# JialeTao/MRFA

Hardware: AMD Instinct MI355X
Metric: frames/sec (256x256 source+driving pair) fwd+bwd (higher is better)
Workload: dtype f32; 1 GPU; vox1.yaml MTIA (TokenPose_B) prior + DenseMotion + RaftFlow refinement, 256x256, bs=8/GPU, fwd+bwd+clip+Adam, train-mode BN, surrogate L1 loss; global_batch=8, parallelism=dp1, prior=mtia, background_predictor=False, sync_bn=False, launch=hipGraph, optimizer=FlatAdam (K20), mfma=bf16x6

## Files before the change

### mrfa_amd/csrc/common.h

```cpp
#pragma once
#include <hip/hip_runtime.h>
#include <stdio.h>
#include <string.h>
#include "mrfa_hip.h"

typedef float f32x16 __attribute__((ext_vector_type(16)));
typedef float f32x4 __attribute__((ext_vector_type(4)));

void mrfa_set_error(const char* fmt, ...);

struct MrfaTuning {
    int conv_small_env;
    int conv_small;
    int conv_halo, conv_halo_min_tiles, conv_halo_pr, conv_halo_phase, conv_halo_bn256, conv_halo_bn192, conv_halo_bn64_fill;
    int conv_lean, conv_lean_min_wgs, conv_lean_geo, gemm_lean;
    int wgrad_halo, wgrad_halo_min_wgs, wgrad_halo_target_wgs, wgrad_halo_phase, wgrad_lean;
    int conv_fewout3, attention_mfma, split_target_256;
};
extern MrfaTuning g_tune;

struct HaloGeo { int PR, BN; bool phase; };

enum class ConvFamily { lean, gemm_lean, small, halo, halo_dgrad, rows_split, rows_f32, refused };
struct ConvPlan {
    ConvFamily family;
    char error[256];
    long long M;
    int KT;
    int lean_geo, gemm_cfg, small_tm, small_tn;
    HaloGeo halo;
    int BM, BN, splitk;
    bool w8;
// ... 175 lines not shown
```

### mrfa_amd/csrc/conv_plan.hip

```cpp
#include "common.h"
#include <stdarg.h>
#include <stdlib.h>

namespace {
int env_int(const char* name, int dflt) { const char* e = getenv(name); return e ? atoi(e) : dflt; }
int env_on(const char* name) { const char* e = getenv(name); return !(e && e[0] == '0'); }
}

MrfaTuning g_tune = {
     env_on("MRFA_CONV_SMALL"),  1,
     env_on("MRFA_CONV_HALO"),  128,  0,  1,  1,
     1,  1,
     env_on("MRFA_CONV_LEAN"),  128,  -1,
     env_int("MRFA_GEMM_LEAN", 1),
     env_on("MRFA_WGRAD_HALO"),  192,  256,  1,
     env_on("MRFA_WGRAD_LEAN"),
     1,  env_on("MRFA_ATTENTION_MFMA"),  env_int("MRFA_SPLIT_TARGET_256", 1),
};

enum TuneKind { T_ON, T_INT, T_NONNEG, T_NONNEG_ON, T_LEVEL, T_POS };
static const struct { const char* key; int* field; TuneKind kind; } TUNING_KEYS[] = {
    {"conv_small", &g_tune.conv_small, T_ON},
    {"conv_halo", &g_tune.conv_halo, T_ON},
    {"conv_halo_min_tiles", &g_tune.conv_halo_min_tiles, T_INT},
    {"conv_halo_pr", &g_tune.conv_halo_pr, T_INT},
    {"conv_halo_phase", &g_tune.conv_halo_phase, T_ON},
    {"conv_halo_bn256", &g_tune.conv_halo_bn256, T_ON},
    {"conv_halo_bn192", &g_tune.conv_halo_bn192, T_ON},
    {"conv_halo_bn64_fill", &g_tune.conv_halo_bn64_fill, T_ON},
    {"conv_lean", &g_tune.conv_lean, T_ON},
    {"conv_lean_min_wgs", &g_tune.conv_lean_min_wgs, T_NONNEG},
    {"conv_lean_geo", &g_tune.conv_lean_geo, T_INT},
    {"gemm_lean", &g_tune.gemm_lean, T_LEVEL},
    {"wgrad_halo", &g_tune.wgrad_halo, T_ON},
    {"wgrad_halo_min_wgs", &g_tune.wgrad_halo_min_wgs, T_NONNEG},
    {"wgrad_halo_target_wgs", &g_tune.wgrad_halo_target_wgs, T_POS},
    {"wgrad_halo_phase", &g_tune.wgrad_halo_phase, T_NONNEG_ON},
    {"wgrad_lean", &g_tune.wgrad_lean, T_ON},
    {"conv_fewout3", &g_tune.conv_fewout3, T_ON},
    {"attention_mfma", &g_tune.attention_mfma, T_ON},
};

extern "C" int mrfa_set_tuning(const char* key, int value) {
    if (!key) return -1;
    for (const auto& k : TUNING_KEYS) {
        if (strcmp(key, k.key)) continue;
        const int prev = *k.field;
        switch (k.kind) {
            case T_ON: *k.field = value != 0; break;
            case T_INT: *k.field = value; break;
            case T_NONNEG: if (value >= 0) *k.field = value; break;
            case T_NONNEG_ON: if (value >= 0) *k.field = value != 0; break;
            case T_LEVEL: if (value >= 0) *k.field = value > 2 ? 2 : value; break;
            case T_POS: if (value > 0) *k.field = value; break;
        }
// ... 202 lines not shown
```

### mrfa_amd/csrc/elementwise.hip

```cpp
#include "common.h"

namespace {

#define GRID_STRIDE(i, total) \
    for (long long i = blockIdx.x * (long long)blockDim.x + threadIdx.x; i < (total); i += (long long)gridDim.x * blockDim.x)

__global__ void avgpool2_fwd_kernel(const float* __restrict__ x, int ldx, int H, int W, int C, float* __restrict__ y, int ldy,
                                    long long total) {
    const int Ho = H / 2, Wo = W / 2;
    GRID_STRIDE(i, total) {
        const long long opix = i / C;
        const int c = (int)(i - opix * C);
        const int ox = (int)(opix % Wo);
        const long long t = opix / Wo;
        const int oy = (int)(t % Ho);
        const long long n = t / Ho;
        const size_t b = (((size_t)n * H + 2 * oy) * W + 2 * ox) * ldx + c;
        y[(size_t)opix * ldy + c] = 0.25f * (x[b] + x[b + ldx] + x[b + (size_t)W * ldx] + x[b + (size_t)(W + 1) * ldx]);
    }
}

__global__ void sumpool2_acc_kernel(const float* __restrict__ x, int ldx, int Ho, int Wo, int C, float* __restrict__ y, int ldy, float mul,
                                    long long total) {
    const int H = 2 * Ho, W = 2 * Wo;
// ... 99 lines not shown
            const float o = occ[(size_t)r * ldo];
            const float g = dy[(size_t)r * lddy + c];
            const float av = a[(size_t)r * lda + c];
            const float bv = b ? b[(size_t)r * ldb + c] : 0.f;
            if (da) da[(size_t)r * ldda + c] += g * o;
            if (db) db[(size_t)r * lddb + c] += g * (1.f - o);
            part = g * (av - bv);
        }
        if (docc) {
            part = wave_sum(part);
            if (lane == 0) atomicAdd(docc + (size_t)r * lddo, part);
        }
    }
}

__global__ __launch_bounds__(256) void colsum_kernel(const float* __restrict__ x, int ldx, long long rows, int C, float* __restrict__ out,
                                                    int rows_per_block) {
    __shared__ float red[4][64];
    const int lane = threadIdx.x & 63, wave = threadIdx.x >> 6;
    const int c = blockIdx.x * 64 + lane;
    const long long r0 = (long long)blockIdx.y * rows_per_block, r1 = min(rows, r0 + rows_per_block);
    float s = 0.f;
    if (c < C)
        for (long long r = r0 + wave; r < r1; r += 4) s += x[(size_t)r * ldx + c];
    red[wave][lane] = s;
    __syncthreads();
    if (wave == 0 && c < C) atomicAdd(out + c, red[0][lane] + red[1][lane] + red[2][lane] + red[3][lane]);
}

__global__ void antialias_kernel(const float* __restrict__ x, int C, int H, int W, const float* __restrict__ kern, int k, int stride,
// ... 77 lines not shown
}

extern "C" int mrfa_blend_fwd(void* stream, const float* a, int lda, const float* b, int ldb, const float* occ, int ldo, long long rows,
                              int C, float* y, int ldy) {
    MRFA_CHECK_ARG(a && occ && y && rows > 0 && C > 0, "blend_fwd: bad args");
    const long long total = rows * C;
    hipLaunchKernelGGL(blend_fwd_kernel, dim3(stream_grid(total, 256)), dim3(256), 0, (hipStream_t)stream, a, lda, b, ldb, occ, ldo, C, y,
                       ldy, total);
    MRFA_CHECK_LAUNCH("blend_fwd");
    return 0;
}

extern "C" int mrfa_blend_bwd(void* stream, const float* a, int lda, const float* b, int ldb, const float* occ, int ldo, const float* dy,
                              int lddy, long long rows, int C, float* da, int ldda, float* db, int lddb, float* docc, int lddo) {
    MRFA_CHECK_ARG(a && occ && dy && rows > 0 && C > 0, "blend_bwd: bad args");
    const long long waves = rows * cdiv(C, 64);
    hipLaunchKernelGGL(blend_bwd_kernel, dim3(stream_grid(waves * 64, 256)), dim3(256), 0, (hipStream_t)stream, a, lda, b, ldb, occ, ldo, dy,
                       lddy, rows, C, da, ldda, db, lddb, docc, lddo);
    MRFA_CHECK_LAUNCH("blend_bwd");
    return 0;
}

extern "C" int mrfa_colsum(void* stream, const float* x, int ldx, long long rows, int C, float* out) {
    MRFA_CHECK_ARG(x && out && rows > 0 && C > 0, "colsum: bad args");
    const int chunks = cdiv(C, 64);
    long long want = (1024 + chunks - 1) / chunks;
    long long rpb = (rows + want - 1) / want;
    if (rpb < 64) rpb = 64;
    dim3 grid(chunks, cdiv(rows, rpb));
    hipLaunchKernelGGL(colsum_kernel, grid, dim3(256), 0, (hipStream_t)stream, x, ldx, rows, C, out, (int)rpb);
// ... 15 lines not shown
```

### mrfa_amd/csrc/norm.hip

```cpp
#include "common.h"

namespace {

constexpr int CH = 64;
constexpr int NW = 4;

__global__ __launch_bounds__(256) void bn_stats_kernel(const float* __restrict__ x, int ldx, long long rows, int C,
                                                      double* __restrict__ stats, int rows_per_block) {
    __shared__ float red[2][NW][CH];
    const int lane = threadIdx.x & 63, wave = threadIdx.x >> 6;
    const int c = blockIdx.x * CH + lane;
    const long long r0 = (long long)blockIdx.y * rows_per_block;
    const long long r1 = min(rows, r0 + rows_per_block);
    float s1 = 0.f, s2 = 0.f;
    if (c < C) {
        for (long long r = r0 + wave; r < r1; r += NW) {
            const float v = x[(size_t)r * ldx + c];
            s1 += v;
            s2 += v * v;
        }
    }
    red[0][wave][lane] = s1;
    red[1][wave][lane] = s2;
    __syncthreads();
    if (wave == 0 && c < C) {
        double a = 0.0, b = 0.0;
        for (int w = 0; w < NW; ++w) { a += red[0][w][lane]; b += red[1][w][lane]; }
        double* st = stats + (size_t)((blockIdx.y + blockIdx.x) % MRFA_STATS_SLOTS) * 2 * C;
        atomicAdd(st + c, a);
        atomicAdd(st + C + c, b);
    }
}

__global__ void bn_finalize_kernel(const double* __restrict__ stats, long long count, const float* __restrict__ gamma,
                                   const float* __restrict__ beta, float* __restrict__ rmean, float* __restrict__ rvar,
                                   float momentum, float eps, int C, int train, int groups, float* __restrict__ scale,
                                   float* __restrict__ shift, float* __restrict__ mean_out, float* __restrict__ invstd_out) {
    chain_prio();
    const int c = blockIdx.x * blockDim.x + threadIdx.x;
    if (c >= C) return;
    float rm = rmean ? rmean[c] : 0.f, rv = rvar ? rvar[c] : 0.f;
    for (int g = 0; g < groups; ++g) {
        float mean, invstd;
        if (train) {
            const double* sg = stats + (size_t)g * MRFA_STATS_SLOTS * 2 * C;
// ... 64 lines not shown
    for (long long i = blockIdx.x * (long long)blockDim.x + threadIdx.x; i < total4; i += (long long)gridDim.x * blockDim.x) {
        const long long opix = i / c4;
        const int c = (int)(i - opix * c4) * 4;
        const int gc = gpix ? (int)(opix / gpix) * p.C + c : c;
        const f32x4 sc = *reinterpret_cast<const f32x4*>(p.scale + gc), sh = *reinterpret_cast<const f32x4*>(p.shift + gc);
        f32x4 v = *reinterpret_cast<const f32x4*>(p.x + (size_t)opix * p.ldx + c) * sc + sh;
        if (RES) v += *reinterpret_cast<const f32x4*>(p.res + (size_t)opix * p.ldr + c);
        if (p.relu) {
#pragma unroll
            for (int k = 0; k < 4; ++k) v[k] = fmaxf(v[k], 0.f);
        }
        *reinterpret_cast<f32x4*>(p.y + (size_t)opix * p.ldy + c) = v;
    }
}

__device__ __forceinline__ int red_slots(unsigned row_blocks) {
    return row_blocks >= 64 ? MRFA_STATS_SLOTS : (row_blocks >= 16 ? 8 : 1);
}

struct GroupSpan {
    int g;
    unsigned by, row_blocks;
    long long cnt, r0, r1;
};
__device__ __forceinline__ GroupSpan group_span(const mrfa_bnbwd_params& p, long long rows, int rows_per_block) {
    GroupSpan s;
    const int G = p.groups > 1 ? p.groups : 1;
    s.row_blocks = gridDim.y / G;
    s.g = blockIdx.y / s.row_blocks;
    s.by = blockIdx.y - s.g * s.row_blocks;
// ... 78 lines not shown
    if (PHASE == 1) {
        red[0][wave][lane] = s1;
        red[1][wave][lane] = s2;
        __syncthreads();
        if (wave == 0 && c_ok) {
            double a = 0.0, b = 0.0;
            for (int w = 0; w < NW; ++w) { a += red[0][w][lane]; b += red[1][w][lane]; }
            double* rd = red_g + (size_t)((gs.by + blockIdx.x) % red_slots(gs.row_blocks)) * 2 * p.C;
            atomicAdd(rd + c, a);
            atomicAdd(rd + p.C + c, b);
        }
    }
}


template <int PHASE, int MODE>
__device__ __forceinline__ void bn_bwd_body(const mrfa_bnbwd_params& p, long long rows, int rows_per_block, float (&red)[2][16][CH],
                                            double (&redsum)[2][CH]) {
    constexpr bool POOL = MODE == 2, BLEND = MODE == 3, RES = MODE == 1;
    const int lane = threadIdx.x & 63, wave = threadIdx.x >> 6;
    const int cg = lane & 15, rsub = lane >> 4;
    const int slot = wave * 4 + rsub;
    const int c = blockIdx.x * CH + cg * 4;
    const bool c_ok = c < p.C;
    const GroupSpan gs = group_span(p, rows, rows_per_block);
    const int gc = gs.g * p.C + c;
    double* const red_g = p.red + (size_t)gs.g * MRFA_STATS_SLOTS * 2 * p.C;
    if (PHASE == 2 && (p.train || p.dbeta || p.dgamma)) {
        const int nslots = p.red_all ? MRFA_STATS_SLOTS : red_slots(gs.row_blocks);
        const int q = threadIdx.x & 3, col = (threadIdx.x >> 2) & 63;
        const int cc = blockIdx.x * CH + col;
// ... 72 lines not shown
                    if (st) {
#pragma unroll
                        for (int k = 0; k < 4; ++k) {
                            s1[k] += du[k];
                            s2[k] += du[k] * (xv[u][k] - mean[k]) * invstd[k];
                        }
                    }
                } else if (st) {
#pragma unroll
                    for (int k = 0; k < 4; ++k)
                        cur[u][k] += p.train ? gi[k] * (du[k] - k1[k] - (xv[u][k] - mean[k]) * invstd[k] * k2[k]) : du[k] * sc[k];
                    *reinterpret_cast<f32x4*>(p.dx + (size_t)rr[u] * p.lddx + c) = cur[u];
                }
            }
        }
    } else
    for (long long r = r0 + slot; r < r1; r += 16) {
        long long opix = r;
        float gmul = 1.f;
        if (POOL) {
            const int xx = (int)(r % p.W);
            const long long t = r / p.W;
            const int yy = (int)(t % p.H);
            const long long n = t / p.H;
            opix = ((long long)n * Ho + (yy >> 1)) * Wo + (xx >> 1);
            gmul = 0.25f;
        }
        f32x4 du = {0, 0, 0, 0}, xv = du;
        float docc_part = 0.f;
        if (c_ok) {
// ... 66 lines not shown
            red[0][slot][cg * 4 + k] = s1[k];
            red[1][slot][cg * 4 + k] = s2[k];
        }
        __syncthreads();
        const int cc = blockIdx.x * CH + threadIdx.x;
        if (threadIdx.x < CH && cc < p.C) {
            double a = 0.0, b = 0.0;
            for (int w = 0; w < 16; ++w) { a += red[0][w][threadIdx.x]; b += red[1][w][threadIdx.x]; }
            double* rd = red_g + (size_t)((gs.by + blockIdx.x) % red_slots(gs.row_blocks)) * 2 * p.C;
            atomicAdd(rd + cc, a);
            atomicAdd(rd + p.C + cc, b);
        }
    }
}

template <int PHASE, int MODE>
__global__ __launch_bounds__(256) void bn_act_bwd_vec_kernel(const mrfa_bnbwd_params p, long long rows, int rows_per_block) {
    chain_prio();
    __shared__ float red[2][16][CH];
    __shared__ double redsum[2][CH];
    bn_bwd_body<PHASE, MODE>(p, rows, rows_per_block, red, redsum);
}

__global__ void bn_param_grad_kernel(const double* __restrict__ red, float* __restrict__ dgamma, float* __restrict__ dbeta, int C, int nslots) {
    chain_prio();
    const int c = blockIdx.x * blockDim.x + threadIdx.x;
    if (c >= C) return;
    double t1 = 0.0, t2 = 0.0;
    for (int s = 0; s < nslots; ++s) { t1 += red[(size_t)s * 2 * C + c]; t2 += red[(size_t)s * 2 * C + C + c]; }
    if (dbeta) atomicAdd(dbeta + c, (float)t1);
    if (dgamma) atomicAdd(dgamma + c, (float)t2);
}

extern "C" int mrfa_bn_param_grad_groups(void* stream, const double* red, int C, int groups, float* dgamma, float* dbeta) {
    MRFA_CHECK_ARG(red && C > 0 && groups >= 1 && (dgamma || dbeta), "bn_param_grad: bad args");
    hipLaunchKernelGGL(bn_param_grad_kernel, dim3(cdiv(C, 256)), dim3(256), 0, (hipStream_t)stream, red, dgamma, dbeta, C, groups * MRFA_STATS_SLOTS);
// ... 11 lines not shown
    if (target > 1024) target = 1024;
    long long want = (target + chunks - 1) / chunks;
    long long rpb = (rows + want - 1) / want;
    if (rpb < 64) rpb = 64;
    if (rpb > 4096) rpb = 4096;
    return (int)rpb;
}

}

extern "C" int mrfa_bn_stats(void* stream, const float* x, int ldx, long long rows, int C, double* stats) {
    MRFA_CHECK_ARG(x && stats && rows > 0 && C > 0, "bn_stats: bad args");
    const int chunks = cdiv(C, CH);
    const int rpb = pick_rows_per_block(rows, chunks, C);
    dim3 grid(chunks, cdiv(rows, rpb));
    hipLaunchKernelGGL(bn_stats_kernel, grid, dim3(256), 0, (hipStream_t)stream, x, ldx, rows, C, stats, rpb);
    MRFA_CHECK_LAUNCH("bn_stats");
    return 0;
}

extern "C" int mrfa_bn_finalize(void* stream, const double* stats, long long count, const float* gamma, const float* beta,
                                float* running_mean, float* running_var, float momentum, float eps, int C, int train,
                                float* scale, float* shift, float* mean_out, float* invstd_out) {
    MRFA_CHECK_ARG(gamma && beta && scale && shift && C > 0, "bn_finalize: bad args");
    MRFA_CHECK_ARG(train ? stats != nullptr : (running_mean && running_var), "bn_finalize: missing statistics");
    hipLaunchKernelGGL(bn_finalize_kernel, dim3(cdiv(C, 256)), dim3(256), 0, (hipStream_t)stream, stats, count, gamma, beta,
                       running_mean, running_var, momentum, eps, C, train, 1, scale, shift, mean_out, invstd_out);
    MRFA_CHECK_LAUNCH("bn_finalize");
    return 0;
}
// ... 14 lines not shown
    MRFA_CHECK_ARG(p.x && p.y && p.scale && p.shift, "bn_act_fwd: null pointer");
    MRFA_CHECK_ARG(!p.pool || ((p.H % 2) == 0 && (p.W % 2) == 0), "bn_act_fwd: pool needs even H,W");
    MRFA_CHECK_ARG(!(p.pool && p.blend_a), "bn_act_fwd: pool and blend are exclusive");
    MRFA_CHECK_ARG(!(p.res && (p.pool || p.blend_a)), "bn_act_fwd: residual excludes pool and blend");
    MRFA_CHECK_ARG(p.groups <= 1 || (p.N % p.groups) == 0, "bn_act_fwd: %d statistic groups do not divide N = %d", p.groups, p.N);
    const long long opix = (long long)p.N * (p.pool ? p.H / 2 : p.H) * (p.pool ? p.W / 2 : p.W);
    const long long total = opix * p.C;
    if (!p.pool && !p.blend_a && (p.C % 4) == 0 && (p.ldx % 4) == 0 && (p.ldy % 4) == 0 && aligned16(p.x) && aligned16(p.y) && aligned16(p.scale) &&
        aligned16(p.shift) && (!p.res || ((p.ldr % 4) == 0 && aligned16(p.res)))) {
        const long long total4 = total / 4;
        if (p.res) hipLaunchKernelGGL((bn_act_fwd_vec_kernel<true>), dim3(stream_grid(total4, 256)), dim3(256), 0, (hipStream_t)stream, p, total4, p.C / 4);
        else hipLaunchKernelGGL((bn_act_fwd_vec_kernel<false>), dim3(stream_grid(total4, 256)), dim3(256), 0, (hipStream_t)stream, p, total4, p.C / 4);
        MRFA_CHECK_LAUNCH("bn_act_fwd(vec)");
        return 0;
    }
    hipLaunchKernelGGL(bn_act_fwd_kernel, dim3(stream_grid(total, 256)), dim3(256), 0, (hipStream_t)stream, p, total);
    MRFA_CHECK_LAUNCH("bn_act_fwd");
    return 0;
}

extern "C" int mrfa_bn_act_bwd(void* stream, const mrfa_bnbwd_params* pp) {
    const mrfa_bnbwd_params& p = *pp;
    MRFA_CHECK_ARG(p.x && p.dy && p.scale && p.shift && p.red, "bn_act_bwd: null pointer");
    MRFA_CHECK_ARG(!p.train || (p.mean && p.invstd && p.gamma), "bn_act_bwd: train mode needs mean/invstd/gamma");
    MRFA_CHECK_ARG(!(p.res && (p.pool || p.blend_a)) && !(p.dres && !p.res), "bn_act_bwd: residual excludes pool and blend");
    MRFA_CHECK_ARG(!(p.pool && p.blend_a), "bn_act_bwd: pool and blend are exclusive (one compile-time MODE per launch)");
    const int G = p.groups > 1 ? p.groups : 1;
    MRFA_CHECK_ARG((p.N % G) == 0, "bn_act_bwd: %d statistic groups do not divide N = %d", G, p.N);
    const long long rows = (long long)p.N * p.H * p.W;
    const int chunks = cdiv(p.C, CH);
    const int rpb = pick_rows_per_block(rows, chunks, p.C);
    dim3 grid(chunks, G * cdiv(rows / G, rpb));
    MRFA_CHECK_ARG(p.phase == 1 || p.phase == 2, "bn_act_bwd: phase %d", p.phase);
    const bool vec = (p.C % 4 == 0) && (p.ldx % 4 == 0) && (p.lddy % 4 == 0) && aligned16(p.x) && aligned16(p.dy) && aligned16(p.scale) &&
                     aligned16(p.shift) && (!p.mean || (aligned16(p.mean) && aligned16(p.invstd))) && (!p.gamma || aligned16(p.gamma)) &&
                     (p.phase == 1 || ((p.lddx % 4 == 0) && aligned16(p.dx))) &&
                     (!p.res || ((p.ldr % 4 == 0) && aligned16(p.res) && (!p.dres || ((p.lddr % 4 == 0) && aligned16(p.dres))))) &&
                     (!p.blend_a || ((p.lda % 4 == 0) && aligned16(p.blend_a) && (!p.dblend_a || ((p.ldda % 4 == 0) && aligned16(p.dblend_a)))));
    if (vec) {
        MRFA_CHECK_ARG(p.phase == 1 || p.dx != nullptr, "bn_act_bwd: phase 2 needs dx");
        const int mode = p.pool ? 2 : (p.blend_a ? 3 : (p.res ? 1 : 0));
#define BNB(PH, MD) hipLaunchKernelGGL((bn_act_bwd_vec_kernel<PH, MD>), grid, dim3(256), 0, (hipStream_t)stream, p, rows, rpb)
        if (p.phase == 1) { if (mode == 0) BNB(1, 0); else if (mode == 1) BNB(1, 1); else if (mode == 2) BNB(1, 2); else BNB(1, 3); }
        else { if (mode == 0) BNB(2, 0); else if (mode == 1) BNB(2, 1); else if (mode == 2) BNB(2, 2); else BNB(2, 3); }
#undef BNB
        MRFA_CHECK_LAUNCH("bn_act_bwd(vec)");
        return 0;
    }
    if (p.phase == 1) {
        hipLaunchKernelGGL((bn_act_bwd_kernel<1>), grid, dim3(256), 0, (hipStream_t)stream, p, rows, rpb);
    } else {
        MRFA_CHECK_ARG(p.dx != nullptr, "bn_act_bwd: phase 2 needs dx");
        hipLaunchKernelGGL((bn_act_bwd_kernel<2>), grid, dim3(256), 0, (hipStream_t)stream, p, rows, rpb);
        if (p.dgamma || p.dbeta) {
            hipLaunchKernelGGL(bn_param_grad_kernel, dim3(cdiv(p.C, 256)), dim3(256), 0, (hipStream_t)stream, p.red, p.dgamma, p.dbeta,
                               p.C, G * MRFA_STATS_SLOTS);
        }
    }
    MRFA_CHECK_LAUNCH("bn_act_bwd");
    return 0;
}
```

### mrfa_amd/csrc/sample.hip

```cpp
#include "mfma_bf16.h"

namespace {

struct Taps {
    int x0, y0;
    float fx, fy;
};

__device__ __forceinline__ Taps make_taps(float ix, float iy) {
    Taps t;
    const float fx0 = floorf(ix), fy0 = floorf(iy);
    t.x0 = (int)fx0;
    t.y0 = (int)fy0;
    t.fx = ix - fx0;
    t.fy = iy - fy0;
    return t;
}


struct Taps4 {
    size_t o00, o01, o10, o11;
    float w00, w01, w10, w11;
    float fx, fy;
    bool ok00, ok01, ok10, ok11;
// ... 276 lines not shown
        const int oy = (int)(t % Ho);
        const long long n = t / Ho;
        int x0, x1, y0, y1;
        float fx, fy;
        resize_src(ox, Wi, Wo, x0, x1, fx);
        resize_src(oy, Hi, Ho, y0, y1, fy);
        const float* b = in + (size_t)n * Hi * Wi * ldi + c;
        const float top = b[((size_t)y0 * Wi + x0) * ldi] * (1.f - fx) + b[((size_t)y0 * Wi + x1) * ldi] * fx;
        const float bot = b[((size_t)y1 * Wi + x0) * ldi] * (1.f - fx) + b[((size_t)y1 * Wi + x1) * ldi] * fx;
        const float v = (top * (1.f - fy) + bot * fy) * mul;
        float* d = out + (size_t)opix * ldo + c;
        *d = acc ? (*d + v) : v;
    }
}

__global__ void resize_bwd_kernel(const float* __restrict__ dout, int lddo, int N, int Hi, int Wi, int C, float* __restrict__ din,
                                  int lddi, int Ho, int Wo, float mul, long long total) {
    for (long long i = blockIdx.x * (long long)blockDim.x + threadIdx.x; i < total; i += (long long)gridDim.x * blockDim.x) {
        const long long opix = i / C;
        const int c = (int)(i - opix * C);
        const int ox = (int)(opix % Wo);
        const long long t = opix / Wo;
        const int oy = (int)(t % Ho);
        const long long n = t / Ho;
        int x0, x1, y0, y1;
        float fx, fy;
        resize_src(ox, Wi, Wo, x0, x1, fx);
        resize_src(oy, Hi, Ho, y0, y1, fy);
        const float g = dout[(size_t)opix * lddo + c] * mul;
        float* b = din + (size_t)n * Hi * Wi * lddi + c;
// ... 22 lines not shown
        for (int oy = oy_lo; oy <= oy_hi; ++oy) {
            int y0, y1; float fy;
            resize_src(oy, Hi, Ho, y0, y1, fy);
            const float wy = (y0 == iy ? 1.f - fy : 0.f) + (y1 == iy ? fy : 0.f);
            if (wy == 0.f) continue;
            float row = 0.f;
            for (int ox = ox_lo; ox <= ox_hi; ++ox) {
                int x0, x1; float fx;
                resize_src(ox, Wi, Wo, x0, x1, fx);
                const float wx = (x0 == ix ? 1.f - fx : 0.f) + (x1 == ix ? fx : 0.f);
                if (wx != 0.f) row += wx * g[((size_t)oy * Wo + ox) * lddo];
            }
            acc += wy * row;
        }
        din[(size_t)ipix * lddi + c] += acc * mul;
    }
}

struct ResizeSumArgs {
    int n;
    int prefix[MRFA_RESIZE_SUM_MAX + 1];
    mrfa_resize_sum_desc d[MRFA_RESIZE_SUM_MAX];
};

template <bool BWD>
__global__ __launch_bounds__(256) void resize_sum_multi_kernel(const ResizeSumArgs a) {
    int lo = 0, hi = a.n;
    while (hi - lo > 1) {
        const int mid = (lo + hi) >> 1;
        if ((int)blockIdx.x >= a.prefix[mid]) lo = mid; else hi = mid;
// ... 291 lines not shown
        dim3 g(stream_grid(npix * C / 4, 256));
#define GSB(L) hipLaunchKernelGGL((grid_sample_bwd_vec_kernel<L>), g, dim3(256), 0, (hipStream_t)stream, in, ldi, in_bstride, in_rep, Hi, Wi, C, \
                                   grid, ldg, npix, Ho, Wo, dout, lddo, mode, din, lddi, din_bstride, dgrid, lddg)
        if (lpp == 64) GSB(64); else if (lpp == 32) GSB(32); else GSB(16);
#undef GSB
        MRFA_CHECK_LAUNCH("grid_sample_bwd(vec)");
        return 0;
    }
    const long long waves = (long long)N * Ho * cdiv(Wo, GS_RUN) * cdiv(C, 64);
    hipLaunchKernelGGL(grid_sample_bwd_kernel, dim3(stream_grid(waves * 64, 256)), dim3(256), 0, (hipStream_t)stream, in, ldi, in_bstride,
                       in_rep, Hi, Wi, C, grid, ldg, npix, Ho, Wo, dout, lddo, mode, din, lddi, din_bstride, dgrid, lddg);
    MRFA_CHECK_LAUNCH("grid_sample_bwd");
    return 0;
}

extern "C" int mrfa_resize_bilinear_fwd(void* stream, const float* in, int ldi, int N, int Hi, int Wi, int C, float* out, int ldo,
                                        int Ho, int Wo, float scale_mul, int accumulate) {
    MRFA_CHECK_ARG(in && out && C > 0 && N > 0 && Hi > 0 && Wi > 0 && Ho > 0 && Wo > 0 && ldi >= C && ldo >= C,
                   "resize_fwd: bad args (sizes must be positive, ldi >= C, ldo >= C; C %d, ldi %d, ldo %d, %d x %d -> %d x %d)", C, ldi, ldo, Hi, Wi, Ho, Wo);
    const long long total = (long long)N * Ho * Wo * C;
    hipLaunchKernelGGL(resize_fwd_kernel, dim3(stream_grid(total, 256)), dim3(256), 0, (hipStream_t)stream, in, ldi, N, Hi, Wi, C, out, ldo,
                       Ho, Wo, scale_mul, accumulate, total);
    MRFA_CHECK_LAUNCH("resize_fwd");
    return 0;
}

extern "C" int mrfa_resize_bilinear_bwd(void* stream, const float* dout, int lddo, int N, int Hi, int Wi, int C, float* din, int lddi,
                                        int Ho, int Wo, float scale_mul) {
    MRFA_CHECK_ARG(dout && din && C > 0 && N > 0 && Hi > 0 && Wi > 0 && Ho > 0 && Wo > 0 && lddo >= C && lddi >= C,
                   "resize_bwd: bad args (sizes must be positive, lddo >= C, lddi >= C; C %d, lddo %d, lddi %d, %d x %d -> %d x %d)", C, lddo, lddi, Hi, Wi, Ho, Wo);
    if (Ho >= Hi && Wo >= Wi) {
        const long long total_in = (long long)N * Hi * Wi * C;
        hipLaunchKernelGGL(resize_bwd_gather_kernel, dim3(stream_grid(total_in, 256)), dim3(256), 0, (hipStream_t)stream, dout, lddo, N, Hi,
                           Wi, C, din, lddi, Ho, Wo, scale_mul, total_in);
        MRFA_CHECK_LAUNCH("resize_bwd_gather");
        return 0;
    }
    const long long total = (long long)N * Ho * Wo * C;
    hipLaunchKernelGGL(resize_bwd_kernel, dim3(stream_grid(total, 256)), dim3(256), 0, (hipStream_t)stream, dout, lddo, N, Hi, Wi, C, din,
                       lddi, Ho, Wo, scale_mul, total);
    MRFA_CHECK_LAUNCH("resize_bwd");
    return 0;
}

static int resize_sum_launch(void* stream, const mrfa_resize_sum_desc* descs, int n, bool bwd, const char* what) {
    MRFA_CHECK_ARG(n >= 0 && (n == 0 || descs), "%s: bad args", what);
    for (int base = 0; base < n; base += MRFA_RESIZE_SUM_MAX) {
// ... 94 lines not shown
```

Before: 103.2 pairs/s.

## Add float4/float2 streaming kernels for BN stats, BN-act, blend bwd and resize

Adds a tuning flag elementwise_vec (on by default) that routes several memory-bound kernels to vectorized variants. These cover float4 BN statistics, a float4 BN-act forward for pool and blend modes, a streaming pool-mode BN backward, a per-row blend backward for C<=4, and float4/float2 bilinear resize forward and gather-backward. The goal is fewer load/store instructions, wider memory transactions and more unrolled loads in flight on these bandwidth-bound ops. Risks are extra register pressure, different FMA rounding, and hard errors when elementwise_vec=2 is set on views that cannot be vectorized.

```diff
diff --git a/mrfa_amd/csrc/common.h b/mrfa_amd/csrc/common.h
--- a/mrfa_amd/csrc/common.h
+++ b/mrfa_amd/csrc/common.h
@@ -16,6 +16,7 @@
     int conv_lean, conv_lean_min_wgs, conv_lean_geo, gemm_lean;
     int wgrad_halo, wgrad_halo_min_wgs, wgrad_halo_target_wgs, wgrad_halo_phase, wgrad_lean;
     int conv_fewout3, attention_mfma, split_target_256;
+    int elementwise_vec;
 };
 extern MrfaTuning g_tune;
 
diff --git a/mrfa_amd/csrc/conv_plan.hip b/mrfa_amd/csrc/conv_plan.hip
--- a/mrfa_amd/csrc/conv_plan.hip
+++ b/mrfa_amd/csrc/conv_plan.hip
@@ -16,6 +16,7 @@
      env_on("MRFA_WGRAD_HALO"),  192,  256,  1,
      env_on("MRFA_WGRAD_LEAN"),
      1,  env_on("MRFA_ATTENTION_MFMA"),  env_int("MRFA_SPLIT_TARGET_256", 1),
+     1,
 };
 
 enum TuneKind { T_ON, T_INT, T_NONNEG, T_NONNEG_ON, T_LEVEL, T_POS };
@@ -39,6 +40,7 @@
     {"wgrad_lean", &g_tune.wgrad_lean, T_ON},
     {"conv_fewout3", &g_tune.conv_fewout3, T_ON},
     {"attention_mfma", &g_tune.attention_mfma, T_ON},
+    {"elementwise_vec", &g_tune.elementwise_vec, T_LEVEL},
 };
 
 extern "C" int mrfa_set_tuning(const char* key, int value) {
diff --git a/mrfa_amd/csrc/elementwise.hip b/mrfa_amd/csrc/elementwise.hip
--- a/mrfa_amd/csrc/elementwise.hip
+++ b/mrfa_amd/csrc/elementwise.hip
@@ -137,6 +137,37 @@
     }
 }
 
+template <int CMAX>
+__global__ __launch_bounds__(256) void blend_bwd_rows_kernel(const float* __restrict__ a, int lda, const float* __restrict__ b, int ldb,
+                                                            const float* __restrict__ occ, int ldo, const float* __restrict__ dy, int lddy,
+                                                            long long rows, int C, float* __restrict__ da, int ldda, float* __restrict__ db,
+                                                            int lddb, float* __restrict__ docc, int lddo) {
+#pragma clang fp contract(off)
+    GRID_STRIDE(r, rows) {
+        float g[CMAX], av[CMAX], bv[CMAX], ca[CMAX], cb[CMAX];
+        const float o = occ[(size_t)r * ldo];
+#pragma unroll
+        for (int c = 0; c < CMAX; ++c) {
+            const int cc = c < C ? c : 0;
+            g[c] = dy[(size_t)r * lddy + cc];
+            av[c] = a[(size_t)r * lda + cc];
+            bv[c] = b ? b[(size_t)r * ldb + cc] : 0.f;
+            ca[c] = da ? da[(size_t)r * ldda + cc] : 0.f;
+            cb[c] = db ? db[(size_t)r * lddb + cc] : 0.f;
+        }
+        float part = 0.f;
+#pragma unroll
+        for (int c = 0; c < CMAX; ++c) {
+            if (c < C) {
+                if (da) da[(size_t)r * ldda + c] = __builtin_fmaf(g[c], o, ca[c]);
+                if (db) db[(size_t)r * lddb + c] = __builtin_fmaf(g[c], 1.f - o, cb[c]);
+                part += g[c] * (av[c] - bv[c]);
+            }
+        }
+        if (docc) atomicAdd(docc + (size_t)r * lddo, part);
+    }
+}
+
 __global__ __launch_bounds__(256) void colsum_kernel(const float* __restrict__ x, int ldx, long long rows, int C, float* __restrict__ out,
                                                     int rows_per_block) {
     __shared__ float red[4][64];
@@ -244,6 +275,14 @@
 extern "C" int mrfa_blend_bwd(void* stream, const float* a, int lda, const float* b, int ldb, const float* occ, int ldo, const float* dy,
                               int lddy, long long rows, int C, float* da, int ldda, float* db, int lddb, float* docc, int lddo) {
     MRFA_CHECK_ARG(a && occ && dy && rows > 0 && C > 0, "blend_bwd: bad args");
+    const int ev = g_tune.elementwise_vec;
+    if (ev && C <= 4) {
+        hipLaunchKernelGGL((blend_bwd_rows_kernel<4>), dim3(stream_grid(rows, 256)), dim3(256), 0, (hipStream_t)stream, a, lda, b, ldb, occ, ldo, dy, lddy,
+                           rows, C, da, ldda, db, lddb, docc, lddo);
+        MRFA_CHECK_LAUNCH("blend_bwd(rows)");
+        return 0;
+    }
+    MRFA_CHECK_ARG(ev != 2, "blend_bwd: only C <= 4 has a streaming kernel (elementwise_vec = 2; C %d)", C);
     const long long waves = rows * cdiv(C, 64);
     hipLaunchKernelGGL(blend_bwd_kernel, dim3(stream_grid(waves * 64, 256)), dim3(256), 0, (hipStream_t)stream, a, lda, b, ldb, occ, ldo, dy,
                        lddy, rows, C, da, ldda, db, lddb, docc, lddo);
diff --git a/mrfa_amd/csrc/norm.hip b/mrfa_amd/csrc/norm.hip
--- a/mrfa_amd/csrc/norm.hip
+++ b/mrfa_amd/csrc/norm.hip
@@ -29,6 +29,46 @@
         double* st = stats + (size_t)((blockIdx.y + blockIdx.x) % MRFA_STATS_SLOTS) * 2 * C;
         atomicAdd(st + c, a);
         atomicAdd(st + C + c, b);
+    }
+}
+
+__global__ __launch_bounds__(256) void bn_stats_vec_kernel(const float* __restrict__ x, int ldx, long long rows, int C,
+                                                          double* __restrict__ stats, int rows_per_block) {
+    __shared__ float red[2][16][CH];
+    const int lane = threadIdx.x & 63, wave = threadIdx.x >> 6;
+    const int cg = lane & 15, slot = wave * 4 + (lane >> 4);
+    const int c = blockIdx.x * CH + cg * 4;
+    const int cl = c < C ? c : 0;
+    const long long r0 = (long long)blockIdx.y * rows_per_block;
+    const long long r1 = min(rows, r0 + rows_per_block);
+    f32x4 s1 = {0, 0, 0, 0}, s2 = s1;
+    for (long long r = r0 + slot; r < r1; r += 64) {
+        f32x4 v[4];
+#pragma unroll
+        for (int u = 0; u < 4; ++u) {
+            const bool live = r + 16 * u < r1;
+            v[u] = *reinterpret_cast<const f32x4*>(x + (size_t)(live ? r + 16 * u : r) * ldx + cl);
+            if (!live) v[u] = f32x4{0.f, 0.f, 0.f, 0.f};
+        }
+#pragma unroll
+        for (int u = 0; u < 4; ++u) {
+            s1 += v[u];
+            s2 += v[u] * v[u];
+        }
+    }
+#pragma unroll
+    for (int k = 0; k < 4; ++k) {
+        red[0][slot][cg * 4 + k] = s1[k];
+        red[1][slot][cg * 4 + k] = s2[k];
+    }
+    __syncthreads();
+    const int cc = blockIdx.x * CH + threadIdx.x;
+    if (threadIdx.x < CH && cc < C) {
+        double a = 0.0, b = 0.0;
+        for (int w = 0; w < 16; ++w) { a += red[0][w][threadIdx.x]; b += red[1][w][threadIdx.x]; }
+        double* st = stats + (size_t)((blockIdx.y + blockIdx.x) % MRFA_STATS_SLOTS) * 2 * C;
+        atomicAdd(st + cc, a);
+        atomicAdd(st + C + cc, b);
     }
 }
 
@@ -123,6 +163,68 @@
     }
 }
 
+template <int MODE>
+__global__ __launch_bounds__(256) void bn_act_fwd_stream_kernel(const mrfa_bnact_params p, unsigned total4, unsigned c4) {
+#pragma clang fp contract(off)
+    chain_prio();
+    constexpr bool POOL = MODE == 2;
+    constexpr int Q = POOL ? 4 : 1;
+    const unsigned Ho = POOL ? p.H / 2 : p.H, Wo = POOL ? p.W / 2 : p.W;
+    const unsigned gpix = p.groups > 1 ? (unsigned)(p.N / p.groups) * Ho * Wo : 0;
+    const unsigned stride = gridDim.x * blockDim.x;
+    for (unsigned i = blockIdx.x * blockDim.x + threadIdx.x; i < total4; i += 2 * stride) {
+        bool live[2];
+        unsigned opix[2], c[2];
+        f32x4 sc[2], sh[2], xv[2][Q], A[2];
+        float o[2];
+#pragma unroll
+        for (int u = 0; u < 2; ++u) {
+            live[u] = i + u * stride < total4;
+            const unsigned ii = live[u] ? i + u * stride : i;
+            opix[u] = ii / c4;
+            c[u] = (ii - opix[u] * c4) * 4;
+            const unsigned gc = gpix ? opix[u] / gpix * (unsigned)p.C + c[u] : c[u];
+            sc[u] = *reinterpret_cast<const f32x4*>(p.scale + gc);
+            sh[u] = *reinterpret_cast<const f32x4*>(p.shift + gc);
+            if (POOL) {
+                const unsigned t = opix[u] / Wo, ox = opix[u] - t * Wo;
+                const unsigned n = t / Ho, oy = t - n * Ho;
+                const size_t base = ((size_t)n * p.H + 2 * oy) * p.W + 2 * ox;
+#pragma unroll
+                for (int q = 0; q < Q; ++q) xv[u][q] = *reinterpret_cast<const f32x4*>(p.x + (base + (q >> 1) * p.W + (q & 1)) * p.ldx + c[u]);
+            } else {
+                xv[u][0] = *reinterpret_cast<const f32x4*>(p.x + (size_t)opix[u] * p.ldx + c[u]);
+                o[u] = p.occ[(size_t)opix[u] * p.ldo];
+                A[u] = *reinterpret_cast<const f32x4*>(p.blend_a + (size_t)opix[u] * p.lda + c[u]);
+            }
+        }
+#pragma unroll
+        for (int u = 0; u < 2; ++u) {
+            f32x4 y;
+#pragma unroll
+            for (int k = 0; k < 4; ++k) {
+                float v;
+                if (POOL) {
+                    float a = 0.f;
+#pragma unroll
+                    for (int q = 0; q < Q; ++q) {
+                        float t = __builtin_fmaf(xv[u][q][k], sc[u][k], sh[u][k]);
+                        if (p.relu) t = fmaxf(t, 0.f);
+                        a += t;
+                    }
+                    v = 0.25f * a;
+                } else {
+                    v = __builtin_fmaf(xv[u][0][k], sc[u][k], sh[u][k]);
+                    if (p.relu) v = fmaxf(v, 0.f);
+                    v = A[u][k] * o[u] + v * (1.f - o[u]);
+                }
+                y[k] = v;
+            }
+            if (live[u]) *reinterpret_cast<f32x4*>(p.y + (size_t)opix[u] * p.ldy + c[u]) = y;
+        }
+    }
+}
+
 __device__ __forceinline__ int red_slots(unsigned row_blocks) {
     return row_blocks >= 64 ? MRFA_STATS_SLOTS : (row_blocks >= 16 ? 8 : 1);
 }
@@ -231,7 +333,7 @@
 }
 
 
-template <int PHASE, int MODE>
+template <int PHASE, int MODE, bool STREAM>
 __device__ __forceinline__ void bn_bwd_body(const mrfa_bnbwd_params& p, long long rows, int rows_per_block, float (&red)[2][16][CH],
                                             double (&redsum)[2][CH]) {
     constexpr bool POOL = MODE == 2, BLEND = MODE == 3, RES = MODE == 1;
@@ -334,6 +436,53 @@
                 }
             }
         }
+    } else if constexpr (STREAM) {
+        static_assert(POOL, "the streaming row loop is the pool mode's");
+        const int cl = c_ok ? c : 0;
+        for (long long r = r0 + slot; r < r1; r += 32) {
+            long long rr[2];
+            bool live[2];
+            f32x4 xv[2], da[2], cur[2];
+#pragma unroll
+            for (int u = 0; u < 2; ++u) {
+                live[u] = r + 16 * u < r1;
+                rr[u] = live[u] ? r + 16 * u : r;
+                const unsigned ur = (unsigned)rr[u], t = ur / (unsigned)p.W, xx = ur - t * (unsigned)p.W;
+                const unsigned n = t / (unsigned)p.H, yy = t - n * (unsigned)p.H;
+                const long long op = ((long long)n * Ho + (yy >> 1)) * Wo + (xx >> 1);
+                xv[u] = *reinterpret_cast<const f32x4*>(p.x + (size_t)rr[u] * p.ldx + cl);
+                da[u] = *reinterpret_cast<const f32x4*>(p.dy + (size_t)op * p.lddy + cl);
+                cur[u] = f32x4{0.f, 0.f, 0.f, 0.f};
+                if (PHASE == 2 && !p.dx_overwrite) cur[u] = *reinterpret_cast<const f32x4*>(p.dx + (size_t)rr[u] * p.lddx + cl);
+            }
+#pragma unroll
+            for (int u = 0; u < 2; ++u) {
+                const bool st = c_ok && live[u];
+                const f32x4 rs = {0.f, 0.f, 0.f, 0.f};
+                f32x4 du;
+#pragma unroll
+                for (int k = 0; k < 4; ++k) {
+                    const float uu = xv[u][k] * sc[k] + sh[k] + rs[k];
+                    du[k] = (p.relu && uu <= 0.f) ? 0.f : da[u][k] * 0.25f;
+                }
+                if (PHASE == 1) {
+                    if (st) {
+#pragma unroll
+                        for (int k = 0; k < 4; ++k) {
+                            s1[k] += du[k];
+                            s2[k] += du[k] * (xv[u][k] - mean[k]) * invstd[k];
+                        }
+                    }
+                } else if (st) {
+#pragma unroll
+                    for (int k = 0; k < 4; ++k) {
+                        const float dx = p.train ? gi[k] * (du[k] - k1[k] - (xv[u][k] - mean[k]) * invstd[k] * k2[k]) : du[k] * sc[k];
+                        cur[u][k] += dx;
+                    }
+                    *reinterpret_cast<f32x4*>(p.dx + (size_t)rr[u] * p.lddx + c) = cur[u];
+                }
+            }
+        }
     } else
     for (long long r = r0 + slot; r < r1; r += 16) {
         long long opix = r;
@@ -430,12 +579,12 @@
     }
 }
 
-template <int PHASE, int MODE>
+template <int PHASE, int MODE, bool STREAM = false>
 __global__ __launch_bounds__(256) void bn_act_bwd_vec_kernel(const mrfa_bnbwd_params p, long long rows, int rows_per_block) {
     chain_prio();
     __shared__ float red[2][16][CH];
     __shared__ double redsum[2][CH];
-    bn_bwd_body<PHASE, MODE>(p, rows, rows_per_block, red, redsum);
+    bn_bwd_body<PHASE, MODE, STREAM>(p, rows, rows_per_block, red, redsum);
 }
 
 __global__ void bn_param_grad_kernel(const double* __restrict__ red, float* __restrict__ dgamma, float* __restrict__ dbeta, int C, int nslots) {
@@ -477,6 +626,13 @@
     const int chunks = cdiv(C, CH);
     const int rpb = pick_rows_per_block(rows, chunks, C);
     dim3 grid(chunks, cdiv(rows, rpb));
+    const int ev = g_tune.elementwise_vec;
+    if (ev && (C % 4) == 0 && (ldx % 4) == 0 && aligned16(x)) {
+        hipLaunchKernelGGL(bn_stats_vec_kernel, grid, dim3(256), 0, (hipStream_t)stream, x, ldx, rows, C, stats, rpb);
+        MRFA_CHECK_LAUNCH("bn_stats(vec)");
+        return 0;
+    }
+    MRFA_CHECK_ARG(ev != 2, "bn_stats: the view cannot take the float4 kernel (elementwise_vec = 2; C %d, ldx %d)", C, ldx);
     hipLaunchKernelGGL(bn_stats_kernel, grid, dim3(256), 0, (hipStream_t)stream, x, ldx, rows, C, stats, rpb);
     MRFA_CHECK_LAUNCH("bn_stats");
     return 0;
@@ -521,6 +677,17 @@
         MRFA_CHECK_LAUNCH("bn_act_fwd(vec)");
         return 0;
     }
+    const int ev = g_tune.elementwise_vec;
+    if (ev && (p.pool || p.blend_a) && (p.C % 4) == 0 && (p.ldx % 4) == 0 && (p.ldy % 4) == 0 && aligned16(p.x) && aligned16(p.y) &&
+        aligned16(p.scale) && aligned16(p.shift) && (!p.blend_a || ((p.lda % 4) == 0 && aligned16(p.blend_a) && p.occ)) && total / 4 < (1ll << 31)) {
+        const unsigned total4 = (unsigned)(total / 4);
+        const dim3 grid(stream_grid(((long long)total4 + 1) / 2, 256));
+        if (p.pool) hipLaunchKernelGGL((bn_act_fwd_stream_kernel<2>), grid, dim3(256), 0, (hipStream_t)stream, p, total4, (unsigned)(p.C / 4));
+        else hipLaunchKernelGGL((bn_act_fwd_stream_kernel<3>), grid, dim3(256), 0, (hipStream_t)stream, p, total4, (unsigned)(p.C / 4));
+        MRFA_CHECK_LAUNCH("bn_act_fwd(stream)");
+        return 0;
+    }
+    MRFA_CHECK_ARG(ev != 2, "bn_act_fwd: the views cannot take a float4 kernel (elementwise_vec = 2; C %d, ldx %d, ldy %d)", p.C, p.ldx, p.ldy);
     hipLaunchKernelGGL(bn_act_fwd_kernel, dim3(stream_grid(total, 256)), dim3(256), 0, (hipStream_t)stream, p, total);
     MRFA_CHECK_LAUNCH("bn_act_fwd");
     return 0;
@@ -548,12 +715,19 @@
         MRFA_CHECK_ARG(p.phase == 1 || p.dx != nullptr, "bn_act_bwd: phase 2 needs dx");
         const int mode = p.pool ? 2 : (p.blend_a ? 3 : (p.res ? 1 : 0));
 #define BNB(PH, MD) hipLaunchKernelGGL((bn_act_bwd_vec_kernel<PH, MD>), grid, dim3(256), 0, (hipStream_t)stream, p, rows, rpb)
-        if (p.phase == 1) { if (mode == 0) BNB(1, 0); else if (mode == 1) BNB(1, 1); else if (mode == 2) BNB(1, 2); else BNB(1, 3); }
+#define BNS(PH) hipLaunchKernelGGL((bn_act_bwd_vec_kernel<PH, 2, true>), grid, dim3(256), 0, (hipStream_t)stream, p, rows, rpb)
+        if (mode == 2 && g_tune.elementwise_vec && rows < (1ll << 31)) {
+            if (p.phase == 1) BNS(1); else BNS(2);
+        }
+        else if (p.phase == 1) { if (mode == 0) BNB(1, 0); else if (mode == 1) BNB(1, 1); else if (mode == 2) BNB(1, 2); else BNB(1, 3); }
         else { if (mode == 0) BNB(2, 0); else if (mode == 1) BNB(2, 1); else if (mode == 2) BNB(2, 2); else BNB(2, 3); }
+#undef BNS
 #undef BNB
         MRFA_CHECK_LAUNCH("bn_act_bwd(vec)");
         return 0;
     }
+    MRFA_CHECK_ARG(g_tune.elementwise_vec != 2, "bn_act_bwd: the views cannot take the float4 kernel (elementwise_vec = 2; C %d, ldx %d, lddy %d)", p.C,
+                   p.ldx, p.lddy);
     if (p.phase == 1) {
         hipLaunchKernelGGL((bn_act_bwd_kernel<1>), grid, dim3(256), 0, (hipStream_t)stream, p, rows, rpb);
     } else {
diff --git a/mrfa_amd/csrc/sample.hip b/mrfa_amd/csrc/sample.hip
--- a/mrfa_amd/csrc/sample.hip
+++ b/mrfa_amd/csrc/sample.hip
@@ -314,6 +314,45 @@
     }
 }
 
+typedef float f32x2 __attribute__((ext_vector_type(2)));
+template <int V> struct FVec;
+template <> struct FVec<4> { typedef f32x4 type; };
+template <> struct FVec<2> { typedef f32x2 type; };
+
+template <int V>
+__global__ __launch_bounds__(256) void resize_fwd_stream_kernel(const float* __restrict__ in, int ldi, int Hi, int Wi, int CV, float* __restrict__ out,
+                                                               int ldo, int Ho, int Wo, float mul, int acc, unsigned totalv) {
+#pragma clang fp contract(off)
+    typedef typename FVec<V>::type vec;
+    for (unsigned i = blockIdx.x * blockDim.x + threadIdx.x; i < totalv; i += gridDim.x * blockDim.x) {
+        const unsigned opix = i / (unsigned)CV;
+        const unsigned c = (i - opix * (unsigned)CV) * (unsigned)V;
+        const unsigned t = opix / (unsigned)Wo;
+        const int ox = (int)(opix - t * (unsigned)Wo);
+        const unsigned n = t / (unsigned)Ho;
+        const int oy = (int)(t - n * (unsigned)Ho);
+        int x0, x1, y0, y1;
+        float fx, fy;
+        resize_src(ox, Wi, Wo, x0, x1, fx);
+        resize_src(oy, Hi, Ho, y0, y1, fy);
+        const float* b = in + (size_t)n * Hi * Wi * ldi + c;
+        const vec v00 = *reinterpret_cast<const vec*>(b + ((size_t)y0 * Wi + x0) * ldi), v01 = *reinterpret_cast<const vec*>(b + ((size_t)y0 * Wi + x1) * ldi);
+        const vec v10 = *reinterpret_cast<const vec*>(b + ((size_t)y1 * Wi + x0) * ldi), v11 = *reinterpret_cast<const vec*>(b + ((size_t)y1 * Wi + x1) * ldi);
+        vec* d = reinterpret_cast<vec*>(out + (size_t)opix * ldo + c);
+        vec cur = v00;
+        if (acc) cur = *d;
+        vec r;
+#pragma unroll
+        for (int k = 0; k < V; ++k) {
+            const float top = __builtin_fmaf(v01[k], fx, v00[k] * (1.f - fx));
+            const float bot = __builtin_fmaf(v10[k], 1.f - fx, v11[k] * fx);
+            const float v = (top * (1.f - fy) + bot * fy) * mul;
+            r[k] = acc ? (cur[k] + v) : v;
+        }
+        *d = r;
+    }
+}
+
 __global__ void resize_bwd_kernel(const float* __restrict__ dout, int lddo, int N, int Hi, int Wi, int C, float* __restrict__ din,
                                   int lddi, int Ho, int Wo, float mul, long long total) {
     for (long long i = blockIdx.x * (long long)blockDim.x + threadIdx.x; i < total; i += (long long)gridDim.x * blockDim.x) {
@@ -366,6 +405,56 @@
             acc += wy * row;
         }
         din[(size_t)ipix * lddi + c] += acc * mul;
+    }
+}
+
+template <int V>
+__global__ __launch_bounds__(256) void resize_bwd_gather_stream_kernel(const float* __restrict__ dout, int lddo, int Hi, int Wi, int CV,
+                                                                      float* __restrict__ din, int lddi, int Ho, int Wo, float mul, unsigned totalv) {
+#pragma clang fp contract(off)
+    typedef typename FVec<V>::type vec;
+    const float sy = Ho > 1 ? (float)(Hi - 1) / (float)(Ho - 1) : 0.f, sx = Wo > 1 ? (float)(Wi - 1) / (float)(Wo - 1) : 0.f;
+    for (unsigned i = blockIdx.x * blockDim.x + threadIdx.x; i < totalv; i += gridDim.x * blockDim.x) {
+        const unsigned ipix = i / (unsigned)CV;
+        const unsigned c = (i - ipix * (unsigned)CV) * (unsigned)V;
+        const unsigned t = ipix / (unsigned)Wi;
+        const int ix = (int)(ipix - t * (unsigned)Wi);
+        const unsigned n = t / (unsigned)Hi;
+        const int iy = (int)(t - n * (unsigned)Hi);
+        vec* d = reinterpret_cast<vec*>(din + (size_t)ipix * lddi + c);
+        const vec cur = *d;
+        int oy_lo = sy > 0.f ? (int)floorf((float)(iy - 1) / sy) - 1 : 0, oy_hi = sy > 0.f ? (int)ceilf((float)(iy + 1) / sy) + 1 : Ho - 1;
+        int ox_lo = sx > 0.f ? (int)floorf((float)(ix - 1) / sx) - 1 : 0, ox_hi = sx > 0.f ? (int)ceilf((float)(ix + 1) / sx) + 1 : Wo - 1;
+        oy_lo = max(oy_lo, 0); oy_hi = min(oy_hi, Ho - 1); ox_lo = max(ox_lo, 0); ox_hi = min(ox_hi, Wo - 1);
+        const float* g = dout + (size_t)n * Ho * Wo * lddo + c;
+        vec acc;
+#pragma unroll
+        for (int k = 0; k < V; ++k) acc[k] = 0.f;
+        for (int oy = oy_lo; oy <= oy_hi; ++oy) {
+            int y0, y1; float fy;
+            resize_src(oy, Hi, Ho, y0, y1, fy);
+            const float wy = (y0 == iy ? 1.f - fy : 0.f) + (y1 == iy ? fy : 0.f);
+            if (wy == 0.f) continue;
+            vec row;
+#pragma unroll
+            for (int k = 0; k < V; ++k) row[k] = 0.f;
+            for (int ox = ox_lo; ox <= ox_hi; ++ox) {
+                int x0, x1; float fx;
+                resize_src(ox, Wi, Wo, x0, x1, fx);
+                const float wx = (x0 == ix ? 1.f - fx : 0.f) + (x1 == ix ? fx : 0.f);
+                if (wx != 0.f) {
+                    const vec gv = *reinterpret_cast<const vec*>(g + ((size_t)oy * Wo + ox) * lddo);
+#pragma unroll
+                    for (int k = 0; k < V; ++k) row[k] = __builtin_fmaf(wx, gv[k], row[k]);
+                }
+            }
+#pragma unroll
+            for (int k = 0; k < V; ++k) acc[k] = __builtin_fmaf(wy, row[k], acc[k]);
+        }
+        vec r;
+#pragma unroll
+        for (int k = 0; k < V; ++k) r[k] = __builtin_fmaf(acc[k], mul, cur[k]);
+        *d = r;
     }
 }
 
@@ -687,11 +776,28 @@
     return 0;
 }
 
+static int resize_vec(int C, int lda, int ldb, const void* a, const void* b) {
+    const uintptr_t m = (uintptr_t)C * 4 | (uintptr_t)lda * 4 | (uintptr_t)ldb * 4 | reinterpret_cast<uintptr_t>(a) | reinterpret_cast<uintptr_t>(b);
+    return (m & 15u) == 0 ? 4 : ((m & 7u) == 0 ? 2 : 0);
+}
+
 extern "C" int mrfa_resize_bilinear_fwd(void* stream, const float* in, int ldi, int N, int Hi, int Wi, int C, float* out, int ldo,
                                         int Ho, int Wo, float scale_mul, int accumulate) {
     MRFA_CHECK_ARG(in && out && C > 0 && N > 0 && Hi > 0 && Wi > 0 && Ho > 0 && Wo > 0 && ldi >= C && ldo >= C,
                    "resize_fwd: bad args (sizes must be positive, ldi >= C, ldo >= C; C %d, ldi %d, ldo %d, %d x %d -> %d x %d)", C, ldi, ldo, Hi, Wi, Ho, Wo);
     const long long total = (long long)N * Ho * Wo * C;
+    const int ev = g_tune.elementwise_vec;
+    const int V = ev ? resize_vec(C, ldi, ldo, in, out) : 0;
+    if (V && total / V < (1ll << 31)) {
+        const unsigned totalv = (unsigned)(total / V);
+        if (V == 4) hipLaunchKernelGGL((resize_fwd_stream_kernel<4>), dim3(stream_grid(totalv, 256)), dim3(256), 0, (hipStream_t)stream, in, ldi, Hi, Wi, C / 4,
+                                       out, ldo, Ho, Wo, scale_mul, accumulate, totalv);
+        else hipLaunchKernelGGL((resize_fwd_stream_kernel<2>), dim3(stream_grid(totalv, 256)), dim3(256), 0, (hipStream_t)stream, in, ldi, Hi, Wi, C / 2,
+                                out, ldo, Ho, Wo, scale_mul, accumulate, totalv);
+        MRFA_CHECK_LAUNCH("resize_fwd(stream)");
+        return 0;
+    }
+    MRFA_CHECK_ARG(ev != 2, "resize_fwd: the views cannot take a vector kernel (elementwise_vec = 2; C %d, ldi %d, ldo %d)", C, ldi, ldo);
     hipLaunchKernelGGL(resize_fwd_kernel, dim3(stream_grid(total, 256)), dim3(256), 0, (hipStream_t)stream, in, ldi, N, Hi, Wi, C, out, ldo,
                        Ho, Wo, scale_mul, accumulate, total);
     MRFA_CHECK_LAUNCH("resize_fwd");
@@ -704,6 +810,18 @@
                    "resize_bwd: bad args (sizes must be positive, lddo >= C, lddi >= C; C %d, lddo %d, lddi %d, %d x %d -> %d x %d)", C, lddo, lddi, Hi, Wi, Ho, Wo);
     if (Ho >= Hi && Wo >= Wi) {
         const long long total_in = (long long)N * Hi * Wi * C;
+        const int ev = g_tune.elementwise_vec;
+        const int V = ev ? resize_vec(C, lddo, lddi, dout, din) : 0;
+        if (V && total_in / V < (1ll << 31)) {
+            const unsigned totalv = (unsigned)(total_in / V);
+            if (V == 4) hipLaunchKernelGGL((resize_bwd_gather_stream_kernel<4>), dim3(stream_grid(totalv, 256)), dim3(256), 0, (hipStream_t)stream, dout, lddo,
+                                           Hi, Wi, C / 4, din, lddi, Ho, Wo, scale_mul, totalv);
+            else hipLaunchKernelGGL((resize_bwd_gather_stream_kernel<2>), dim3(stream_grid(totalv, 256)), dim3(256), 0, (hipStream_t)stream, dout, lddo,
+                                    Hi, Wi, C / 2, din, lddi, Ho, Wo, scale_mul, totalv);
+            MRFA_CHECK_LAUNCH("resize_bwd_gather(stream)");
+            return 0;
+        }
+        MRFA_CHECK_ARG(ev != 2, "resize_bwd: the views cannot take a vector kernel (elementwise_vec = 2; C %d, lddo %d, lddi %d)", C, lddo, lddi);
         hipLaunchKernelGGL(resize_bwd_gather_kernel, dim3(stream_grid(total_in, 256)), dim3(256), 0, (hipStream_t)stream, dout, lddo, N, Hi,
                            Wi, C, din, lddi, Ho, Wo, scale_mul, total_in);
         MRFA_CHECK_LAUNCH("resize_bwd_gather");
```

Measured after the change: 102.8 pairs/s. Within noise of the previous version (-0.4%).
